# jamesonquinn/Mamba.jl

Hardware: AMD Instinct MI355X
Metric: chain-updates/sec (iters×chains) on rats model at 1/2/4/8 MI355X (higher is better)
Workload: dtype f64

## Files before the change

mamba.jl_amd/csrc/device.h:

```cpp
#pragma once
#if !defined(__HIPCC_RTC__)
#include <hip/hip_runtime.h>
#include <stdint.h>
#endif

#include "mamba_hip.h"
#include "mmb_math.h"
#include "ir_math.h"

#define MMB_MAXB MMB_MAX_BLOCKS

__device__ __forceinline__ bool mmb_inverse_ballot(uint64_t m) {
#if defined(__HIPCC_RTC__)
  return ((m >> (threadIdx.x & 63)) & 1ull) != 0ull;
#else
  return __builtin_amdgcn_inverse_ballot_w64(m);
#endif
}

template <bool B>
struct mmb_bc {
  static constexpr bool value = B;
  constexpr operator bool() const { return B; }
};

__device__ __forceinline__ bool mmb_fast_range(double x) { return x >= 0x1p-700 && x <= 0x1p700; }
__device__ __forceinline__ double mmb_sqrt_inrange(double x) {
  const double y = __builtin_amdgcn_rsq(x);
  double g = x * y, h = 0.5 * y;
  const double r = fma(-h, g, 0.5);
  g = fma(g, r, g);
  h = fma(h, r, h);
  double d = fma(-g, g, x);
  g = fma(d, h, g);
  d = fma(-g, g, x);
  return fma(d, h, g);
}
__device__ __forceinline__ double mmb_rcp_inrange(double y) {
  double r = __builtin_amdgcn_rcp(y);
  double e = fma(-y, r, 1.0);
  r = fma(r, e, r);
  e = fma(-y, r, 1.0);
  r = fma(r, e, r);
  e = fma(-y, r, 1.0);
  return fma(e, r, r);
}
__device__ __forceinline__ void mmb_sqrt_rcp_inrange(double x, double* s, double* rcp) {
  *s = mmb_sqrt_inrange(x);
  *rcp = mmb_rcp_inrange(*s);
}

#define MMB_AMM_STAT_STRIDE 8

struct DBlock {
  int32_t kind, nn, d, transform, form, adapt, batchsize, sigl_diag;
  int32_t nodes[4];
  int32_t emap[4];
  double target, beta, scale;
  double width0;
  const double* width;
  const double* sigl;
  double* t_sigma;
  double* t_accept;
  int32_t* t_m;
  int32_t* t_flags;
  double* t_Mv;
  double* t_Mvv;
  double* t_Ls;
  uint8_t* t_piv;
  double* t_xnext;
  int64_t* t_xtag;
  uint64_t* t_astat;
  double* t_nuts;
  double* t_nfr;
  double* t_hmc;
  int32_t ir_blk;
  int32_t fdgrad;
  const int32_t* sep;
  double sep_eps;
  int32_t gibbs_fam;
  double gibbs_a;
};

struct SweepArgs {
  int32_t K;
  uint32_t chain_offset;
  uint64_t seed;
  int64_t iter0;
  int32_t n_iters;
  int32_t nb;
  int64_t burnin, thin, model_burnin;
  int64_t kept_base;
  int64_t kept_origin;
  double* vals;
  int64_t xepoch;
  unsigned long long* nuts_stat;
  double* draws;
  const double* data0;
  double ig_c;
  double xbar;
  double xm[5];
  double lx[5], ly[5];
  const DBlock* blocks;
  const mmb_ir_node* ir_nodes;
  const int32_t* ir_code;
  const double* ir_const;
  const double* ir_pool;
  const mmb_ir_block* ir_blocks;
  const int32_t* ir_mon;
  int32_t ir_nmon, ir_pmon;
  int32_t ir_vs;
  int32_t ir_red0;
  int32_t ir_amm;
  int32_t ir_lds;
  const int32_t* cperm;
  int32_t wg_offset;
  int32_t wg_stride;
  int32_t amwg_exact;
  int32_t slice_exact;
  int32_t amwg_probe;
};

#define MMB_ORDER_BLOCKS 3
struct OrderArgs {
  const int32_t* flags[MMB_ORDER_BLOCKS];
  int32_t nblk;
  int32_t K;
  int32_t cpw;
  int32_t mode;
  int32_t* perm;
};

__device__ __forceinline__ const DBlock& mmb_block(const DBlock* p, int b) {
#if defined(__HIP_DEVICE_COMPILE__)
  return *(const DBlock*)&((const __attribute__((address_space(4))) DBlock*)p)[b];
#else
  return p[b];
#endif
}

MMB_HD int mmb_tri(int i) { return (i * (i + 1)) >> 1; }
MMB_HD int mmb_slot(int i, int k) { return i >= k ? mmb_tri(i) + k : mmb_tri(k) + i; }

__device__ __forceinline__ void grp_sync() {
  __builtin_amdgcn_fence(__ATOMIC_RELEASE, "wavefront");
  __builtin_amdgcn_wave_barrier();
  __builtin_amdgcn_fence(__ATOMIC_ACQUIRE, "wavefront");
}

template <int CTRL>
__device__ __forceinline__ int dpp_i(int x) {
  return __builtin_amdgcn_mov_dpp(x, CTRL, 0xF, 0xF, true);
}
template <int CTRL>
__device__ __forceinline__ double dpp_d(double x) {
  uint64_t u = mmb_d2u(x);
  int lo = dpp_i<CTRL>((int)(uint32_t)u), hi = dpp_i<CTRL>((int)(uint32_t)(u >> 32));
  return mmb_u2d((uint64_t)(uint32_t)lo | ((uint64_t)(uint32_t)hi << 32));
}
__device__ __forceinline__ int swap16_i(int x) {
  auto r = __builtin_amdgcn_permlane16_swap((unsigned)x, (unsigned)x, false, false);
  return (int)((threadIdx.x & 16) ? r[0] : r[1]);
}
__device__ __forceinline__ double swap16_d(double x) {
// ... 182 lines not shown
```

mamba.jl_amd/csrc/engine.cpp:

```cpp
#include <hip/hip_runtime.h>

#include <algorithm>
#include <cmath>
#include <cstdarg>
#include <cstdio>
#include <cstdlib>
#include <cstring>
#include <map>
#include <string>
#include <type_traits>
#include <vector>

#include "device.h"
#include "models.h"
#include "nuts.h"
#include "logistic.h"
#include "ir.h"
#include "ir_jit.h"

#include <rccl/rccl.h>

hipError_t mmb_launch_sweep(int model, unsigned kinds, const SweepArgs& A, hipStream_t st);
hipError_t mmb_launch_order_chains(const OrderArgs& a, hipStream_t st);
hipError_t mmb_launch_pchol_probe(int n, int d, const double* S, double* L, int32_t* pos, int32_t* info,
// ... 942 lines not shown
int64_t mmb_num_kept(const mmb_engine* e) { return e ? e->n_kept : MMB_E_ARG; }

int64_t mmb_tune_len(const mmb_engine* e) {
  if (!e) return MMB_E_ARG;
  int64_t n = 0;
  for (auto& h : e->blocks) n += h.tune_len;
  return n;
}

static void to_device_layout(const mmb_engine* e, const double* v, double* dv) {
  if (e->model == MMB_MODEL_RATS) {
    std::fill(dv, dv + e->VS, 0.0);
    for (int i = 0; i < 30; ++i) { dv[i] = v[1 + i]; dv[32 + i] = v[33 + i]; }
    dv[64] = v[0]; dv[65] = v[31]; dv[66] = v[32]; dv[67] = v[63]; dv[68] = v[64];
  } else if (e->model == MMB_MODEL_LOGISTIC || e->model == MMB_MODEL_IR) {
    std::fill(dv, dv + e->VS, 0.0);
    for (int i = 0; i < e->P; ++i) dv[i] = v[i];
  } else {
    dv[0] = v[0]; dv[1] = v[1]; dv[2] = v[2]; dv[3] = 0.0;
  }
}
static void from_device_layout(const mmb_engine* e, const double* dv, double* v) {
  if (e->model == MMB_MODEL_RATS) {
    for (int i = 0; i < 30; ++i) { v[1 + i] = dv[i]; v[33 + i] = dv[32 + i]; }
    v[0] = dv[64]; v[31] = dv[65]; v[32] = dv[66]; v[63] = dv[67]; v[64] = dv[68];
  } else if (e->model == MMB_MODEL_LOGISTIC || e->model == MMB_MODEL_IR) {
    for (int i = 0; i < e->P; ++i) v[i] = dv[i];
  } else {
    v[0] = dv[0]; v[1] = dv[1]; v[2] = dv[2];
  }
}

int mmb_set_values(mmb_engine* e, const double* values) {
  if (!e || !values) return fail(e, MMB_E_ARG, "null argument");
  if (!e->d_vals) return fail(e, MMB_E_STATE, "mmb_init_chains not called");
  ++e->xepoch;
  std::vector<double> h((size_t)e->K * e->VS);
  for (int64_t k = 0; k < e->K; ++k) to_device_layout(e, values + k * e->P, h.data() + k * e->VS);
  HIPCHK(e, hipSetDevice(e->device));
  HIPCHK(e, hipMemcpy(e->d_vals, h.data(), h.size() * sizeof(double), hipMemcpyHostToDevice));
  return 0;
}

int mmb_get_values(mmb_engine* e, double* values) {
  if (!e || !values) return fail(e, MMB_E_ARG, "null argument");
  if (!e->d_vals) return fail(e, MMB_E_STATE, "mmb_init_chains not called");
  std::vector<double> h((size_t)e->K * e->VS);
  HIPCHK(e, hipSetDevice(e->device));
  HIPCHK(e, hipStreamSynchronize(e->stream));
  HIPCHK(e, hipMemcpy(h.data(), e->d_vals, h.size() * sizeof(double), hipMemcpyDeviceToHost));
  for (int64_t k = 0; k < e->K; ++k) from_device_layout(e, h.data() + k * e->VS, values + k * e->P);
  return 0;
}

static int upload_blocks(mmb_engine* e) {
  std::vector<DBlock> db(e->blocks.size());
  for (size_t b = 0; b < e->blocks.size(); ++b) {
    BlockHost& h = e->blocks[b];
    DBlock& d = db[b];
    std::memset(&d, 0, sizeof d);
    d.kind = h.spec.sampler;
    d.nn = h.spec.nnodes;
    d.d = h.d;
    d.transform = h.spec.sampler == MMB_SAMPLER_SLICE ? h.spec.transform : 1;
    d.form = h.spec.form;
    d.adapt = h.spec.adapt;
    d.batchsize = h.spec.batchsize;
    d.sigl_diag = h.sigl_diag;
    d.fdgrad = h.spec.gradient != MMB_GRAD_ANALYTIC ? 1 : 0;
    for (int a = 0; a < 4; ++a) d.nodes[a] = a < h.spec.nnodes ? h.spec.nodes[a] : -1;
    int o = 0;
    for (int a = 0; a < h.spec.nnodes && o < 4; ++a) {
      int n = h.spec.nodes[a];
      if (e->model == MMB_MODEL_LINE) {
        if (n == MMB_LINE_BETA) { d.emap[o++] = 0; if (o < 4) d.emap[o++] = 1; }
        else d.emap[o++] = 2;
      } else {
        d.emap[o++] = n;
      }
    }
    d.target = h.spec.target;
    d.beta = h.spec.beta;
    d.scale = h.spec.scale;
    d.width0 = h.tuning.empty() ? 0.0 : h.tuning[0];
    d.width = (h.spec.sampler == MMB_SAMPLER_SLICE && h.tuning.size() > 1) ? h.width : nullptr;
    d.sigl = h.sigl_d;
    d.t_sigma = h.sigma; d.t_accept = h.accept; d.t_m = h.m; d.t_flags = h.flags;
    d.t_Mv = h.Mv; d.t_Mvv = h.Mvv; d.t_Ls = h.Ls; d.t_piv = h.piv; d.t_xnext = h.xnext; d.t_xtag = h.xtag; d.t_nuts = h.nuts; d.t_nfr = h.nfr;
    d.t_astat = h.astat;
    d.t_hmc = h.hmc;
    d.ir_blk = (int32_t)b;
    d.gibbs_a = __builtin_nan("");
    if (e->model == MMB_MODEL_IR && h.spec.sampler == MMB_SAMPLER_GIBBS) {
      const mmb_ir_block& IB = e->ir_blocks[b];
      const int pc = IB.gibbs_expr[0];
      if (IB.gibbs_family != MMB_IR_NORMAL && pc >= 0 && pc + 1 < (int)e->ir_code.size() &&
          (int)((uint32_t)e->ir_code[pc] >> 24) == MMB_IR_OP_CONST && e->ir_code[pc + 1] == MMB_IR_OP_END) {
        const double a = e->ir_const[e->ir_code[pc] & 0xffffff];
        if (a >= 1.0) d.gibbs_a = a;
      }
      d.gibbs_fam = IB.gibbs_family;
    }
    d.sep = h.sep_d;
    d.sep_eps = h.sep_eps;
  }
  if (!e->d_blocks) HIPCHK(e, hipMalloc(&e->d_blocks, MMB_MAX_BLOCKS * sizeof(DBlock)));
  HIPCHK(e, hipMemcpy(e->d_blocks, db.data(), db.size() * sizeof(DBlock), hipMemcpyHostToDevice));
  return 0;
}

template <class T>
static hipError_t dalloc(T** p, size_t n) {
  return hipMalloc((void**)p, std::max<size_t>(n, 1) * sizeof(T));
}

int mmb_init_chains(mmb_engine* e, const double* init, int64_t K, int64_t chain_offset, uint64_t seed) {
  if (!e || !init) return fail(e, MMB_E_ARG, "null argument");
  if (K < 1 || K > (int64_t)1 << 30) return fail(e, MMB_E_ARG, "K out of range");
  if (chain_offset < 0 || chain_offset + K > ((int64_t)1 << 32))
    return fail(e, MMB_E_ARG, "global chain ids must fit in 32 bits");
  if (!e->have_data) return fail(e, MMB_E_STATE, "inputs must be set before inits");
  HIPCHK(e, hipSetDevice(e->device));
  HIPCHK(e, hipStreamSynchronize(e->stream));
  free_dev(e);
  e->K = K;
  e->chain_offset = chain_offset;
  e->seed = seed;
  e->iter = 0;
  e->n_kept = 0;
  HIPCHK(e, dalloc(&e->d_vals, (size_t)K * e->VS));
  e->slice_overflows = 0;
  HIPCHK(e, dalloc(&e->d_nstat, 8));
  HIPCHK(e, hipMemset(e->d_nstat, 0, 8 * sizeof(unsigned long long)));
  const size_t DP = e->DP, TP = e->TP;
  for (auto& h : e->blocks) {
    HIPCHK(e, dalloc(&h.m, K));
    HIPCHK(e, dalloc(&h.flags, K));
    HIPCHK(e, hipMemset(h.m, 0, K * sizeof(int32_t)));
    HIPCHK(e, hipMemset(h.flags, 0, K * sizeof(int32_t)));
    if (h.spec.sampler == MMB_SAMPLER_AMWG) {
      HIPCHK(e, dalloc(&h.sigma, K * DP));
      HIPCHK(e, dalloc(&h.accept, K * DP));
      std::vector<double> sg(K * DP, 0.0);
      for (int64_t k = 0; k < K; ++k)
        for (int i = 0; i < h.d; ++i) sg[k * DP + i] = h.tuning.size() == 1 ? h.tuning[0] : h.tuning[i];
      HIPCHK(e, hipMemcpy(h.sigma, sg.data(), sg.size() * sizeof(double), hipMemcpyHostToDevice));
      HIPCHK(e, hipMemset(h.accept, 0, K * DP * sizeof(double)));
    } else if (h.spec.sampler == MMB_SAMPLER_AMM) {
      HIPCHK(e, dalloc(&h.Mv, K * DP));
      HIPCHK(e, dalloc(&h.Mvv, K * TP));
      HIPCHK(e, dalloc(&h.Ls, K * TP));
      HIPCHK(e, dalloc(&h.piv, K * DP));
      HIPCHK(e, hipMemset(h.Mv, 0, K * DP * sizeof(double)));
      HIPCHK(e, hipMemset(h.Mvv, 0, K * TP * sizeof(double)));
      HIPCHK(e, hipMemset(h.Ls, 0, K * TP * sizeof(double)));
      std::vector<uint8_t> pv(K * DP);
      for (int64_t k = 0; k < K; ++k)
        for (size_t i = 0; i < DP; ++i) pv[k * DP + i] = (uint8_t)i;
      HIPCHK(e, hipMemcpy(h.piv, pv.data(), pv.size(), hipMemcpyHostToDevice));
      HIPCHK(e, dalloc(&h.xnext, K * DP));
      HIPCHK(e, dalloc(&h.xtag, K));
      HIPCHK(e, hipMemset(h.xtag, 0xff, K * sizeof(int64_t)));
      HIPCHK(e, dalloc(&h.astat, K * MMB_AMM_STAT_STRIDE));
      HIPCHK(e, hipMemset(h.astat, 0, K * MMB_AMM_STAT_STRIDE * sizeof(uint64_t)));
      HIPCHK(e, dalloc(&h.sigl_d, (size_t)h.d * h.d));
      HIPCHK(e, hipMemcpy(h.sigl_d, h.sigl.data(), h.sigl.size() * sizeof(double), hipMemcpyHostToDevice));
// ... 1639 lines not shown
```

mamba.jl_amd/csrc/samplers.h:

```cpp
#pragma once
#include "models.h"
#include "hmc.h"
#include "nuts.h"

template <class M>
struct Smp {
  static constexpr int G = M::G, R = M::R, DMAX = M::DMAX, DP = M::DP, TP = M::TP;
  static constexpr int NT = (TP + G - 1) / G;
  using St = typename M::St;
  using Lc = typename M::Lc;

  __device__ __forceinline__ static double predraw(const SweepArgs& A, uint32_t chain, int64_t it,
                                                   const Grp<G>& g) {
    int q = 0;
    for (int t = A.nb; A.nb > 0 && t + A.nb <= 32; t += A.nb) q += g.lane >= t ? 1 : 0;
    const int bl = g.lane - q * A.nb;
    int kind = 0;
    double a = 0.0;
    for (int b = 0; b < A.nb; ++b) {
      const DBlock& B = mmb_block(A.blocks, b);
      double ab = 0.0;
      int k = 0;
      if (B.kind == MMB_SAMPLER_GIBBS) k = M::gibbs_draw_kind(B, &ab);
      else if (B.kind == MMB_SAMPLER_AMM) k = 3;
// ... 221 lines not shown
          grp_sync();
#pragma unroll
          for (int r = 0; r < R; ++r) {
            int e = r * G + g.lane;
            if (!done[r]) {
              double t0 = 0.0, t1 = 0.0;
#pragma unroll
              for (int k = 0; k + 1 < j; k += 2) {
                const double2 pp = *(const double2*)(prow + k);
                t0 = fma(Lrow[r][k], pp.x, t0);
                t1 = fma(Lrow[r][k + 1], pp.y, t1);
              }
              if (j & 1) t0 = fma(Lrow[r][j - 1], prow[j - 1], t0);
              double lij = (mat[mmb_slot(e, p)] - (t0 + t1)) * rinv;
              Lrow[r][j] = lij;
              work[r] = work[r] + lij * lij;
            }
          }
          grp_sync();
        }
      }
    }
    if (rank == d) {
#pragma unroll
      for (int r = 0; r < R; ++r) {
        int e = r * G + g.lane;
        if (e < d) {
          bool before = true;
#pragma unroll
          for (int k = 0; k < DMAX; ++k) {
            if (k < d) {
              const int q = pks[k];
              if (q == e) {
                mat[mmb_tri(e) + e] = Lrow[r][k];
                before = false;
              } else if (before) {
                mat[mmb_slot(e, q)] = Lrow[r][k];
              }
            }
          }
        }
      }
    }
    return rank;
  }

  __device__ __forceinline__ static int pivot_exact(double dl, bool done, const int* pks, int j,
                                                              int d, int* perm, double* val) {
    const int lane = (int)(threadIdx.x & (G - 1));
    if (lane == 0) {
      for (int t = 0; t < d; ++t) perm[t] = t;
      for (int k = 0; k < j; ++k) {
        int q = pks[k], qpos = k;
        for (int t = k; t < d; ++t) if (perm[t] == q) qpos = t;
        int tmp = perm[k]; perm[k] = q; perm[qpos] = tmp;
      }
    }
    grp_sync();
    int mypos = 0x7fffffff;
    for (int t = j; t < d; ++t) if (perm[t] == lane) mypos = t;
    grp_sync();
    double key = done ? -__builtin_inf()
                      : (isnan(dl) ? (mypos == j ? __builtin_inf() : -__builtin_inf()) : dl);
    int pi = (done ? 0x7fff : mypos) << 16 | lane;
    Grp<G> g;
    g.argmax(key, pi);
    const int p = pi & 0xffff;
    *val = g.bcast(dl, p);
    return p;
  }

  __device__ __forceinline__ static int gmax_i32(int x) {
    x = max(x, dpp_i<MMB_DPP_XOR1>(x));
    x = max(x, dpp_i<MMB_DPP_XOR2>(x));
    x = max(x, dpp_i<MMB_DPP_HMIRROR>(x));
    x = max(x, dpp_i<MMB_DPP_MIRROR>(x));
    auto r = __builtin_amdgcn_permlane16_swap((unsigned)x, (unsigned)x, false, false);
    return max((int)r[0], (int)r[1]);
  }

  __device__ __forceinline__ static int pchol32(int d, double* mat, double* prow, int* pks, const Grp<G>& g,
                                                int* pos_out, const DBlock* NB = nullptr,
                                                const SweepArgs& A = SweepArgs{}, int c = 0, uint32_t chain = 0,
                                                int64_t it = 0, int b = 0, int m = 0, int* redo = nullptr) {
    if (d == DMAX)
      return pchol32_impl<true>(d, mat, prow, pks, pos_out, NB, A.seed, A.xepoch, c, chain, it, b, m, redo);
    return pchol32_impl<false>(d, mat, prow, pks, pos_out, NB, A.seed, A.xepoch, c, chain, it, b, m, redo);
  }
  template <bool FULLD>
  __device__ __forceinline__ static int pchol32_impl(int d_arg, double* mat, double* prow, int* pks, int* pos_out,
                                                     const DBlock* NB, uint64_t seed, int64_t xepoch, int c,
                                                     uint32_t chain, int64_t it, int b, int m,
                                                     int* redo_out) {
    const int d = FULLD ? DMAX : d_arg;
    const Grp<G> g;
    constexpr int RI = DMAX;
    const int lane = g.lane;
    const bool hi_half = (threadIdx.x & 32) != 0;
    const bool inb = lane < d;
    const int lc = inb ? lane : 0;
    const double diag0 = inb ? mat[mmb_tri(lane) + lane] : 0.0;
    double work = 0.0;
    double Lrow[DMAX];
#pragma unroll
    for (int k = 0; k < DMAX; ++k) Lrow[k] = 0.0;
    MMB_PROF_START
    bool done = !inb;
    int rank = d;
    int pe = 0;
    bool live = true;
    auto tail = [&]() __attribute__((always_inline)) -> int {
      MMB_PROF_MARK(10, lane)
      if (NB != nullptr && (rank == d || m <= 2 * d)) {
        const mmb_rng rn1 = mmb_rng_make(seed, chain, (uint32_t)(it + 1), (uint32_t)b, MMB_SUB_NORMAL);
        double z1n = 0.0, z2n = 0.0;
        if (inb) mmb_normal_pair(&rn1, (uint32_t)lane, &z1n, &z2n);
        double a = 0.0;
        if (inb) a = fma(NB->sigl[lane * d + lane], z1n, a);
        if (m > 2 * d) {
          double y = 0.0;
          const double zs = swap16_d(z2n);
          const bool row0 = (lane & 16) == 0;
          const double zA = row0 ? z2n : zs, zB = row0 ? zs : z2n;
#pragma unroll
          for (int k = 0; k < DMAX; ++k) fmac_rowbc_n(y, k < 16 ? zA : zB, Lrow[k], k & 15);
          a = NB->beta * a + (1.0 - NB->beta) * y;
        }
        if (inb) NB->t_xnext[(size_t)c * DP + lane] = a;
        if (lane == 0) NB->t_xtag[c] = (xepoch << 32) | (int64_t)(uint32_t)(it + 1);
      }
      MMB_PROF_MARK(11, lane)
      if (rank == d && inb) {
        const int base = mmb_tri(pe);
#pragma unroll
        for (int k = 0; k < DMAX; ++k) {
          double* dst = k <= pe ? mat + base + k : prow + lane;
          *dst = Lrow[k];
        }
      }
      MMB_PROF_MARK(12, lane)
      *pos_out = pe;
      return rank;
    };
    if (!inb) work = __builtin_inf();
    const uint32_t mat_lds = (uint32_t)(uintptr_t)(__attribute__((address_space(3))) double*)mat;
    int hmask = hi_half ? -1 : 0;
    asm volatile("" : "+v"(hmask));
    constexpr int KEY_LO = 0x14300000;
    constexpr double BIG = 0x1p700;
    auto pass = [&](auto checked_c) __attribute__((always_inline)) -> bool {
      constexpr bool CHECKED = decltype(checked_c)::value;
      double apiv = 1.0;
      double inf_s = __builtin_inf();
      asm volatile("" : "+s"(inf_s));
#pragma unroll
      for (int j = 0; j < DMAX; ++j) {
        if (live && j < d) {
          const double dl = diag0 - work;
          const int key = (int)(mmb_d2u(dl) >> 32);
          const int mx = gmax_i32(key);
          const uint64_t eq = __ballot(key == mx);
          uint32_t elo = (uint32_t)eq, ehi = (uint32_t)(eq >> 32);
          int p = 0;
          const uint64_t negm = __ballot(mx < 0);
          bool pos = mmb_inverse_ballot(~negm);
          bool fast = true;
          if constexpr (!CHECKED) {
            const int plo = __builtin_ctz(elo | 0x80000000u), phi = __builtin_ctz(ehi | 0x80000000u);
            p = plo ^ ((plo ^ phi) & hmask);
          } else {
            const uint64_t act = __builtin_amdgcn_read_exec();
            const uint64_t bad = __ballot(!(dl < BIG));
            const uint64_t big = __ballot(key >= KEY_LO);
            const uint64_t neg = __ballot(mx < 0);
            uint32_t alo = (uint32_t)act, ahi = (uint32_t)(act >> 32);
            uint32_t nlo = (uint32_t)neg, nhi = (uint32_t)(neg >> 32), blo = (uint32_t)big, bhi = (uint32_t)(big >> 32);
            asm("" : "+s"(elo), "+s"(ehi), "+s"(alo), "+s"(ahi));
            asm("" : "+s"(nlo), "+s"(nhi), "+s"(blo), "+s"(bhi));
            const bool ok_lo = alo == 0 || nlo != 0 || ((elo & (elo - 1)) == 0 && blo != 0);
            const bool ok_hi = ahi == 0 || nhi != 0 || ((ehi & (ehi - 1)) == 0 && bhi != 0);
            fast = bad == 0 && ok_lo && ok_hi;
            if (fast) {
              const int plo = __builtin_ctz(elo | 0x80000000u), phi = __builtin_ctz(ehi | 0x80000000u);
              p = plo ^ ((plo ^ phi) & hmask);
            } else {
              double val;
              p = pivot_exact(dl, done, pks, j, d, (int*)prow, &val);
              pos = val > 0.0;
            }
          }
          if (CHECKED && !pos) {
            live = false;
          } else {
            const bool piv = CHECKED ? lane == p : mmb_inverse_ballot(eq & ~negm);
            if (piv) {
              if constexpr (CHECKED) pks[j] = p;
              else apiv = dl;
              if (j + 1 < d) {
#pragma unroll
                for (int k = 0; k + 1 < j; k += 2) *(double2*)(prow + k) = make_double2(Lrow[k], Lrow[k + 1]);
                if (j & 1) prow[j - 1] = Lrow[j - 1];
              }
              double ajj, rinv;
              if (fast) {
                mmb_sqrt_rcp_inrange(dl, &ajj, &rinv);
              } else {
                ajj = sqrt(dl);
                rinv = 1.0 / ajj;
              }
              prow[RI] = rinv;
              Lrow[j] = ajj;
              pe = j;
// ... 23 lines not shown
                }
              }
              const double lij = (sig - (t0 + t1)) * rinv;
              const bool keep = CHECKED ? done : work == inf_s;
              work = work + lij * lij;
              if (!keep) Lrow[j] = lij;
            }
            grp_sync();
            if (!CHECKED) live = live && pos;
          }
        }
      }
      if constexpr (CHECKED) {
        return false;
      } else {
        done = work == inf_s;
        const bool inr = apiv >= 0x1p-700 && apiv <= 0x1p700;
        uint64_t need = __ballot(inb && (done ? !inr : isnan(diag0 - work)));
        const uint64_t dn = __ballot(done && inb);
        const int mpe = gmax_i32((done && inb) ? pe : -1);
        const uint64_t act = __builtin_amdgcn_read_exec();
        const int m0 = __builtin_amdgcn_readlane(mpe, 0), m1 = __builtin_amdgcn_readlane(mpe, 32);
        if ((uint32_t)act != 0u && __builtin_popcount((uint32_t)dn) != m0 + 1) need |= 1ull;
        if ((act >> 32) != 0u && __builtin_popcount((uint32_t)(dn >> 32)) != m1 + 1) need |= 1ull << 32;
        return need != 0;
      }
    };
    if (__builtin_expect(pass(mmb_bc<false>{}), 0)) {
      if (redo_out) *redo_out = 1;
      work = inb ? 0.0 : __builtin_inf();
#pragma unroll
      for (int k = 0; k < DMAX; ++k) Lrow[k] = 0.0;
      done = !inb;
      pe = 0;
      live = true;
      (void)pass(mmb_bc<true>{});
    }
    const uint64_t dn = __ballot(done && inb);
    rank = __builtin_popcount(hi_half ? (uint32_t)(dn >> 32) : (uint32_t)dn);
    return tail();
  }

  static constexpr bool IKTAB = (G == 32);
  __device__ __forceinline__ static uint16_t* ik_table() {
    __shared__ uint16_t tab[IKTAB ? TP : 1];
    return tab;
  }
  __device__ __forceinline__ static void ik_fill() {
    if constexpr (IKTAB) {
      for (int t = (int)threadIdx.x; t < TP; t += (int)blockDim.x) {
        int i, k;
        slot_ik(t, i, k);
        ik_table()[t] = (uint16_t)(i << 8 | k);
      }
    }
  }
  __device__ __forceinline__ static void slot_ik(int s, int& i, int& k) {
    int ii = (int)((sqrtf((float)(8 * s + 1)) - 1.0f) * 0.5f);
    ii += (mmb_tri(ii + 1) <= s) ? 1 : 0;
    ii -= (mmb_tri(ii) > s) ? 1 : 0;
    i = ii;
    k = s - mmb_tri(ii);
  }

  __device__ __forceinline__ static void amm_count(const DBlock& B, int c, int d, int rank, int redo,
                                                   const Grp<G>& g) {
    const int st = rank < d ? rank + 1 : d;
    int ws = st;
    if constexpr (G == 32) {
      const uint64_t act = __builtin_amdgcn_read_exec();
      const int s0 = __builtin_amdgcn_readlane(st, 0), s1 = __builtin_amdgcn_readlane(st, 32);
      ws = max((uint32_t)act != 0u ? s0 : 0, (act >> 32) != 0u ? s1 : 0);
    }
    if (g.lane == 0) {
      uint64_t* a = B.t_astat + (size_t)c * MMB_AMM_STAT_STRIDE;
      (void)__hip_atomic_fetch_add(a + 0, (uint64_t)1, __ATOMIC_RELAXED, __HIP_MEMORY_SCOPE_AGENT);
      if (rank == d) (void)__hip_atomic_fetch_add(a + 1, (uint64_t)1, __ATOMIC_RELAXED, __HIP_MEMORY_SCOPE_AGENT);
      (void)__hip_atomic_fetch_add(a + 2, (uint64_t)rank, __ATOMIC_RELAXED, __HIP_MEMORY_SCOPE_AGENT);
      (void)__hip_atomic_fetch_add(a + 3, (uint64_t)ws, __ATOMIC_RELAXED, __HIP_MEMORY_SCOPE_AGENT);
      if (redo) (void)__hip_atomic_fetch_add(a + 4, (uint64_t)redo, __ATOMIC_RELAXED, __HIP_MEMORY_SCOPE_AGENT);
    }
  }

  static constexpr bool CARRY = (G == 32 && R == 1);
  static constexpr bool POSFORM = (G == 32 && R == 1);
  __device__ __forceinline__ static int64_t xtag(const SweepArgs& A, int64_t it) {
    return (A.xepoch << 32) | (int64_t)(uint32_t)it;
  }
  __device__ __forceinline__ static void amm(const SweepArgs& A, const DBlock& B, int c, uint32_t chain,
                             int64_t it, int b, const mmb_rng& rn,
                             const mmb_rng& ru, bool adapt, St& s, const Lc& l, const Grp<G>& g,
                             double* lds, double upre, typename M::PrepCache& pk) {
    const int d = B.d;
    const int T = mmb_tri(d);
    double* mat = lds;
    double* z2s = lds + TP;
    double* vvs = z2s + DP;
    double* mvs = vvs + DP;
    int* ia = (int*)(mvs + DP);
    double v[R], x[R], z1[R], z2[R], mv[R];
    MMB_PROF_START
    M::unlist(B, s, g.lane, v);
    int m = B.t_m[c];
    int fl = B.t_flags[c];
#pragma unroll
    for (int r = 0; r < R; ++r) {
      int e = r * G + g.lane;
      mv[r] = e < d ? B.t_Mv[(size_t)c * DP + e] : 0.0;
    }
    const bool fresh = adapt && !(fl & 1);
    bool carried = false;
    if constexpr (CARRY) carried = B.t_xtag != nullptr && !fresh && B.t_xtag[c] == xtag(A, it);
    if (fresh) {
      m = 0;
      fl = (fl | 2) & ~4;
#pragma unroll
      for (int r = 0; r < R; ++r) mv[r] = v[r];
    }
    fl = adapt ? (fl | 1) : (fl & ~1);
    MMB_PROF_MARK(1, g.lane)
    if (carried) {
#pragma unroll
      for (int r = 0; r < R; ++r) {
        const int e = r * G + g.lane;
        x[r] = e < d ? B.t_xnext[(size_t)c * DP + e] : 0.0;
      }
    } else {
#pragma unroll
    for (int r = 0; r < R; ++r) {
      int e = r * G + g.lane;
      if (e < d) mmb_normal_pair(&rn, (uint32_t)e, &z1[r], &z2[r]);
      else { z1[r] = 0.0; z2[r] = 0.0; }
    }
    if (!B.sigl_diag) {
#pragma unroll
      for (int r = 0; r < R; ++r) {
        int e = r * G + g.lane;
        if (e < d) vvs[e] = z1[r];
      }
      grp_sync();
    }
#pragma unroll
    for (int r = 0; r < R; ++r) {
      int e = r * G + g.lane;
      double a = 0.0;
      if (e < d) {
        if (B.sigl_diag) {
          a = fma(B.sigl[e * d + e], z1[r], a);
        } else {
          for (int k = 0; k <= e; ++k) a = fma(B.sigl[e * d + k], vvs[k], a);
        }
      }
      x[r] = a;
    }
    if (m > 2 * d) {
      double y[R];
#pragma unroll
      for (int r = 0; r < R; ++r) y[r] = 0.0;
      if (fl & 4) {
        grp_sync();
        const double* Ls = B.t_Ls + (size_t)c * TP;
        double lt[NT];
#pragma unroll
        for (int u = 0; u < NT; ++u) lt[u] = (u * G + g.lane < T) ? Ls[u * G + g.lane] : 0.0;
#pragma unroll
        for (int u = 0; u < NT; ++u)
          if (u * G + g.lane < T) mat[u * G + g.lane] = lt[u];
        if constexpr (POSFORM) {
          const int e = g.lane;
          const int pe = e < d ? (int)B.t_piv[(size_t)c * DP + e] : 0;
          if (e < d) z2s[e] = z2[0];
          grp_sync();
          const double* row = mat + mmb_tri(pe);
          double a = 0.0;
#pragma unroll
          for (int k = 0; k < DMAX; ++k)
            if (k < d) a = k <= pe ? fma(row[k], z2s[k], a) : a;
          if (e < d) y[0] = a;
        } else {
        uint32_t pw[DP / 4];
        const uint32_t* pvw = (const uint32_t*)(B.t_piv + (size_t)c * DP);
#pragma unroll
        for (int w = 0; w < DP / 4; ++w) pw[w] = pvw[w];
#pragma unroll
        for (int r = 0; r < R; ++r) {
          int e = r * G + g.lane;
          if (e < d) z2s[e] = z2[r];
        }
        grp_sync();
#pragma unroll
        for (int r = 0; r < R; ++r) {
          const int e = r * G + g.lane;
          int pe = 0;
#pragma unroll
          for (int k = 0; k < DMAX; ++k)
            if (k < d && (int)((pw[k >> 2] >> (8 * (k & 3))) & 0xffu) == e) pe = k;
          double a = 0.0;
#pragma unroll
          for (int k = 0; k < DMAX; ++k) {
            if (k < d) {
              const int q = (int)((pw[k >> 2] >> (8 * (k & 3))) & 0xffu);
              const double m_ = mat[mmb_slot(e, q)];
              const double z_ = z2s[k];
              a = (k < pe) ? fma(m_, z_, a) : a;
            }
          }
          if (e < d) y[r] = fma(mat[mmb_tri(e) + e], z2s[pe], a);
        }
        }
      }
#pragma unroll
      for (int r = 0; r < R; ++r) x[r] = B.beta * x[r] + (1.0 - B.beta) * y[r];
    }
    }
#pragma unroll
    for (int r = 0; r < R; ++r) x[r] = x[r] + v[r];
    MMB_PROF_MARK(2, g.lane)
    const typename M::Prep pc = M::prep(B, s, g, pk);
    MMB_PROF_MARK(0, g.lane)
    double lx, lv;
    M::logf_p2(A, B, pc, s, l, g, x, v, lx, lv);
    const double ua = G == 32 ? upre : mmb_uniform(&ru, 0u);
    if (ua < mmb_exp(lx - lv)) {
#pragma unroll
      for (int r = 0; r < R; ++r) v[r] = x[r];
    }
    MMB_PROF_MARK(3, g.lane)
    if (adapt) {
      m += 1;
      const double p = (double)m / ((double)m + 1.0);
      const double q = 1.0 - p;
      if (fl & 2) {
#pragma unroll
        for (int r = 0; r < R; ++r) mv[r] = p * v[r] + q * v[r];
        fl &= ~2;
      } else {
#pragma unroll
        for (int r = 0; r < R; ++r) mv[r] = p * mv[r] + q * v[r];
      }
      grp_sync();
      double2* vm = (double2*)vvs;
#pragma unroll
      for (int r = 0; r < R; ++r) {
        int e = r * G + g.lane;
        if (e < d) vm[e] = make_double2(v[r], mv[r]);
      }
      const double cc = (B.scale * B.scale / (double)d) / p;
      double* Mvv = B.t_Mvv + (size_t)c * TP;
      double vold[R];
      if (fresh) {
        M::unlist(B, s, g.lane, vold);
#pragma unroll
        for (int r = 0; r < R; ++r) {
          int e = r * G + g.lane;
          if (e < d) z2s[e] = vold[r];
        }
      }
      grp_sync();
      double lt[NT];
#pragma unroll
      for (int u = 0; u < NT; ++u) lt[u] = (!fresh && u * G + g.lane < TP) ? Mvv[u * G + g.lane] : 0.0;
      double* const Mvv_l = Mvv + g.lane;
      double* const mat_l = mat + g.lane;
      auto slots = [&](auto fresh_c) {
        constexpr bool FRESH = decltype(fresh_c)::value;
        int li0 = g.lane;
        asm volatile("" : "+v"(li0));
#pragma unroll
        for (int u = 0; u < NT; ++u) {
          const int t = u * G + g.lane;
          if ((u + 1) * G <= TP || t < TP) {
            int i, k;
            if constexpr (IKTAB) {
              const int li = li0;
              const int w = ik_table()[li + u * G];
              i = w >> 8;
              k = w & 255;
            } else {
              int ti = t;
              asm volatile("" : "+v"(ti));
              slot_ik(ti, i, k);
            }
            const double2 a = vm[k], bi = vm[i];
            const double old = FRESH ? z2s[i] * z2s[k] : lt[u];
            const double nv = p * old + (q * a.x) * bi.x;
            lt[u] = nv;
            mat_l[u * G] = cc * (nv - a.y * bi.y);
          }
        }
      };
      if (fresh) slots(mmb_bc<true>{});
      else slots(mmb_bc<false>{});
#pragma unroll
      for (int u = 0; u < NT; ++u)
        if ((u + 1) * G <= TP || u * G + g.lane < TP) Mvv_l[u * G] = lt[u];
      grp_sync();
#pragma unroll
      for (int r = 0; r < R; ++r) {
        int e = r * G + g.lane;
        if (e < d) B.t_Mv[(size_t)c * DP + e] = mv[r];
      }
      if (g.lane == 0) { B.t_m[c] = m; B.t_flags[c] = fl; }
      M::relist(B, s, g, v);
      M::stash(lds, s, g.lane);
      int* pks = (int*)z2s;
      grp_sync();
      MMB_PROF_MARK(4, g.lane)
      int rank;
      int redo = 0;
      const bool carry = CARRY && B.t_xtag != nullptr && B.sigl_diag;
      int pe = 0;
      if constexpr (G == 32 && R == 1)
        rank = pchol32(d, mat, (double*)ia, pks, g, &pe, carry ? &B : nullptr, A, c, chain, it, b, m, &redo);
      else
        rank = pchol(d, mat, (double*)ia, pks, g);
      grp_sync();
      MMB_PROF_MARK(5, g.lane)
      if (B.t_astat != nullptr) amm_count(B, c, d, rank, redo, g);
      if (rank == d) {
        double* Ls = B.t_Ls + (size_t)c * TP;
#pragma unroll
        for (int u = 0; u < NT; ++u)
          if (u * G + g.lane < T) Ls[u * G + g.lane] = mat[u * G + g.lane];
        uint8_t* pv = B.t_piv + (size_t)c * DP;
        if constexpr (POSFORM) {
          if (g.lane < d) pv[g.lane] = (uint8_t)pe;
        } else {
          for (int k = g.lane; k < d; k += G) pv[k] = (uint8_t)pks[k];
        }
        if (g.lane == 0) B.t_flags[c] = fl | 4;
      }
      M::unstash(lds, s, g.lane);
      grp_sync();
      MMB_PROF_MARK(6, g.lane)
      return;
    }
#pragma unroll
    for (int r = 0; r < R; ++r) {
      int e = r * G + g.lane;
      if (e < d) B.t_Mv[(size_t)c * DP + e] = mv[r];
    }
    if (g.lane == 0) { B.t_m[c] = m; B.t_flags[c] = fl; }
    grp_sync();
    M::relist(B, s, g, v);
  }

  __device__ __forceinline__ static void slice_overflow(const SweepArgs& A, const Grp<G>& g) {
    if (g.lane == 0) atomicAdd(&A.nuts_stat[3], 1ull);
  }
  __device__ __forceinline__ static double width(const DBlock& B, int e) {
    return B.width ? B.width[e] : B.width0;
  }
  struct UWin {
    double u;
    uint32_t base;
  };
  __device__ __forceinline__ static double uwin_next(const mmb_rng& ru, UWin& w, uint32_t k, const Grp<G>& g) {
    if (k - w.base >= (uint32_t)G) {
      w.base = k;
      w.u = mmb_uniform(&ru, k + (uint32_t)g.lane);
    }
    const int src = (int)(threadIdx.x & 63 & ~(G - 1)) + (int)(k - w.base);
    return __shfl(w.u, src, 64);
  }
  __device__ __forceinline__ static void slice_uni_cand(const SweepArgs& A, const DBlock& B, const mmb_rng& ru,
                                                        St& s, const Lc& l, const Grp<G>& g, double* lds) {
    constexpr int SD = M::SLICE_CAND_D;
    constexpr int NC = M::SLICE_NC, LPC = 32 / NC;
    constexpr uint32_t LEAD = NC == 2 ? 0x00010001u : NC == 4 ? 0x01010101u : 0x11111111u;
    static_assert(MMB_SLICE_MAX_SHRINK % NC == 0, "rounds of candidates end at the cap");
    const int d = B.d;
    double x[R];
    M::unlist(B, s, g.lane, x);
    typename M::SCtx cx;
    M::slice_cand_prep(A, B, s, l, g, lds, cx);
    double logf0 = M::slice_logf0(A, B, s, l, g, x, cx);
    double lo = 0.0, up = 0.0;
    if (g.lane < d) {
      const double w = width(B, g.lane);
      lo = x[0] - w * mmb_uniform(&ru, (uint32_t)g.lane);
      up = lo + w;
    }
    typename M::SMemo memo;
    double xu[SD], lou[SD], upu[SD];
#pragma unroll
    for (int a = 0; a < SD; ++a) {
      xu[a] = a < d ? g.bcast(x[0], a) : 0.0;
      lou[a] = a < d ? g.bcast(lo, a) : 0.0;
      upu[a] = a < d ? g.bcast(up, a) : 0.0;
    }
    uint32_t k = (uint32_t)d;
    UWin uw{0.0, 0xffffffffu - (uint32_t)G};
    const int q = g.lane / LPC;
    const int gbase = (int)(threadIdx.x & 63) & ~(G - 1);
    for (int e = 0; e < d; ++e) {
      const double p0 = logf0 + mmb_log(uwin_next(ru, uw, k++, g));
      double xo = xu[0], lo_ = lou[0], up_ = upu[0];
#pragma unroll
      for (int a = 1; a < SD; ++a)
        if (a == e) { xo = xu[a]; lo_ = lou[a]; up_ = upu[a]; }
      double xn = 0.0, lfn = 0.0;
      for (uint32_t j0 = 0;; j0 += NC) {
        double cand[NC];
#pragma unroll
        for (int t = 0; t < NC; ++t) {
          const double cv = lo_ + (up_ - lo_) * uwin_next(ru, uw, k + j0 + (uint32_t)t, g);
          cand[t] = cv;
          if (cv < xo) lo_ = cv;
          else up_ = cv;
        }
        double mine = cand[0];
#pragma unroll
        for (int t = 1; t < NC; ++t) mine = q == t ? cand[t] : mine;
        double xv[SD];
#pragma unroll
        for (int a = 0; a < SD; ++a) xv[a] = a == e ? mine : xu[a];
        const double lp = M::slice_cand_logf(A, B, s, cx, xv, g.lane, memo);
        const bool hit = !(lp < p0) && j0 + (uint32_t)q + 1u <= (uint32_t)MMB_SLICE_MAX_SHRINK;
        const uint64_t bal = __ballot(hit && (g.lane & (LPC - 1)) == 0);
        const uint32_t hb = (uint32_t)(bal >> gbase) & LEAD;
        if (hb != 0u) {
          const int qs = __builtin_ctz(hb) / LPC;
          xn = cand[0];
#pragma unroll
          for (int t = 1; t < NC; ++t) xn = qs == t ? cand[t] : xn;
// ... 262 lines not shown
```

mamba.jl_amd/csrc/sweep.h:

```cpp
#pragma once
#include "samplers.h"
#include "ir.h"

#ifdef MMB_PHASE_PROF
extern __device__ unsigned long long mmb_prof[32];
#endif
#ifdef MMB_WAVE_TIMES
#define MMB_WT_MAX 65536
extern __device__ unsigned long long mmb_wt[3 * MMB_WT_MAX];
#endif

#ifndef MMB_SWEEP_WAVES
#define MMB_SWEEP_WAVES 4
#endif
#ifndef MMB_IR_WAVES
#define MMB_IR_WAVES 2
#endif
template <int MODEL>
constexpr int sweep_waves() {
  return MODEL == MMB_MODEL_RATS ? MMB_SWEEP_WAVES : MODEL == MMB_MODEL_IR ? MMB_IR_WAVES : 1;
}

template <int MODEL, unsigned KINDS>
__device__ __forceinline__ void sweep_body(const SweepArgs& A) {
  using M = Mdl<MODEL>;
  using S = Smp<M>;
  constexpr int G = M::G;
  extern __shared__ __attribute__((aligned(16))) double smem[];
  if constexpr ((KINDS >> MMB_SAMPLER_AMM) & 1u) {
    S::ik_fill();
    __syncthreads();
  }
#ifdef MMB_IR_POOL_LDS
  if constexpr (MODEL == MMB_MODEL_IR) {
    double* ps = mmb_ir_pool_s();
    for (int t = (int)threadIdx.x; t < MMB_IR_POOL_LDS; t += (int)blockDim.x) ps[t] = A.ir_pool[t];
    __syncthreads();
  }
#endif
  const unsigned wg = blockIdx.x * (unsigned)A.wg_stride + (unsigned)A.wg_offset;
  const int slot = (int)((wg * blockDim.x + threadIdx.x) / G);
#ifdef MMB_WAVE_TIMES
  const uint64_t _wt0 = __builtin_amdgcn_s_memrealtime();
  const int _wid = (int)((wg * blockDim.x + threadIdx.x) >> 6);
#endif
  if (slot >= A.K) return;
  const int c = A.cperm != nullptr ? A.cperm[slot] : slot;
  Grp<G> g;
  double* lds = smem + (size_t)(threadIdx.x / G) * M::lds_stride(A);
  typename M::St s;
  typename M::Lc l;
  M::load(A, c, g.lane, s, l, lds);
  const uint32_t chain = A.chain_offset + (uint32_t)c;
#ifdef MMB_PHASE_PROF
  if ((threadIdx.x & 63) == 0)
    for (int i = 0; i < 16; ++i) mmb_prof_lds()[i] = 0;
#endif
  constexpr bool PREDRAW = G == 32 && (KINDS & ((1u << MMB_SAMPLER_GIBBS) | (1u << MMB_SAMPLER_AMM))) != 0u;
  int pre0 = 0;
  double pre = 0.0;
  typename M::PrepCache pk = M::prep_cache(lds);
  for (int step = 0; step < A.n_iters; ++step) {
    const int64_t it = A.iter0 + 1 + step;
#ifdef MMB_PHASE_PROF
    const uint64_t _it0 = __builtin_amdgcn_s_memtime();
#endif
    if constexpr (PREDRAW) {
      if (__builtin_expect(pre0 == 0, 0)) {
        MMB_PROF_START
        pre = S::predraw(A, chain, it, g);
        MMB_PROF_MARK(15, g.lane)
      }
    }
    for (int b = 0; b < A.nb; ++b) {
      const DBlock& B = mmb_block(A.blocks, b);
      const mmb_rng rn = mmb_rng_make(A.seed, chain, (uint32_t)it, (uint32_t)b, MMB_SUB_NORMAL);
      const mmb_rng ru = mmb_rng_make(A.seed, chain, (uint32_t)it, (uint32_t)b, MMB_SUB_UNIFORM);
      const bool adapt = B.adapt == MMB_ADAPT_ALL ? true
                         : B.adapt == MMB_ADAPT_BURNIN ? (it <= A.model_burnin) : false;
      switch (B.kind) {
        case MMB_SAMPLER_AMWG:
          if constexpr ((KINDS >> MMB_SAMPLER_AMWG) & 1u) {
            MMB_PROF_START
            S::amwg(A, B, c, rn, ru, adapt, s, l, g, pk);
            MMB_PROF_MARK(13, g.lane)
          }
          break;
        case MMB_SAMPLER_AMM:
          if constexpr ((KINDS >> MMB_SAMPLER_AMM) & 1u) S::amm(A, B, c, chain, it, b, rn, ru, adapt, s, l, g, lds,
                                                                        G == 32 ? S::lane_value(pre, pre0 + b) : 0.0, pk);
          break;
        case MMB_SAMPLER_SLICE:
          if constexpr ((KINDS >> MMB_SAMPLER_SLICE) & 1u) {
            MMB_PROF_START
            if (B.form == MMB_SLICE_UNIVARIATE) S::slice_uni(A, B, ru, s, l, g, lds);
            else S::slice_multi(A, B, ru, s, l, g, lds);
            MMB_PROF_MARK(14, g.lane)
          }
          break;
        case MMB_SAMPLER_NUTS:
          if constexpr ((KINDS >> MMB_SAMPLER_NUTS) & 1u) S::nuts(A, B, c, it, b, s, g);
          break;
        case MMB_SAMPLER_HMC:
          if constexpr ((KINDS >> MMB_SAMPLER_HMC) & 1u) S::template hmc<false>(A, B, c, rn, ru, s, g);
          break;
        case MMB_SAMPLER_MALA:
          if constexpr ((KINDS >> MMB_SAMPLER_MALA) & 1u) S::template hmc<true>(A, B, c, rn, ru, s, g);
          break;
        case MMB_SAMPLER_GIBBS: if constexpr ((KINDS >> MMB_SAMPLER_GIBBS) & 1u) {
          const mmb_rng gn = mmb_rng_make(A.seed, chain, (uint32_t)it, (uint32_t)b, MMB_SUB_GAMMA_N);
          const mmb_rng gu = mmb_rng_make(A.seed, chain, (uint32_t)it, (uint32_t)b, MMB_SUB_GAMMA_U);
          MMB_PROF_START
          M::gibbs(A, B, s, l, g, &rn, &gn, &gu, G == 32 ? S::lane_value(pre, pre0 + b) : 0.0);
          MMB_PROF_MARK(7, g.lane)
        }
          break;
        default:
          break;
      }
      M::prep_wrote(pk, B);
    }
#ifdef MMB_PHASE_PROF
    if ((threadIdx.x & 63) == 0) {
      mmb_prof_lds()[8] += __builtin_amdgcn_s_memtime() - _it0;
      mmb_prof_lds()[9] += 1;
    }
#endif
    pre0 += A.nb;
    if (pre0 + A.nb > 32) pre0 = 0;
    if (A.draws && it > A.burnin && (it - A.burnin) % A.thin == 0) {
      const int64_t row = (it - A.burnin) / A.thin - 1 - A.kept_origin;
      M::write_draws(A, s, g, row, c);
    }
  }
  M::store(A, c, g.lane, s);
#ifdef MMB_WAVE_TIMES
  if ((threadIdx.x & 63) == 0 && _wid < MMB_WT_MAX) {
    const uint64_t _wt1 = __builtin_amdgcn_s_memrealtime();
    if (mmb_wt[3 * _wid] == 0) mmb_wt[3 * _wid] = _wt0;
    mmb_wt[3 * _wid + 1] = _wt1;
    mmb_wt[3 * _wid + 2] += _wt1 - _wt0;
  }
#endif
#ifdef MMB_PHASE_PROF
  if ((threadIdx.x & 63) == 0)
    for (int i = 0; i < 16; ++i) atomicAdd(&mmb_prof[i], mmb_prof_lds()[i]);
#endif
}

#ifndef MMB_RATS_BLOCK
#define MMB_RATS_BLOCK 256
#endif
template <int MODEL, unsigned KINDS>
__global__ __launch_bounds__(MODEL == MMB_MODEL_RATS && MMB_RATS_BLOCK > 256 ? MMB_RATS_BLOCK : 256,
                             sweep_waves<MODEL>()) void sweep_kernel(const SweepArgs A) {
  sweep_body<MODEL, KINDS>(A);
}

constexpr unsigned K_ALL = (1u << MMB_SAMPLER_AMWG) | (1u << MMB_SAMPLER_AMM) |
                         (1u << MMB_SAMPLER_SLICE) | (1u << MMB_SAMPLER_GIBBS);
constexpr unsigned K_GRAD = (1u << MMB_SAMPLER_NUTS) | (1u << MMB_SAMPLER_HMC) | (1u << MMB_SAMPLER_MALA);
constexpr unsigned K_ALL_GRAD = K_ALL | K_GRAD;
constexpr unsigned K_GIBBS_AMM = (1u << MMB_SAMPLER_AMM) | (1u << MMB_SAMPLER_GIBBS);
constexpr unsigned K_SLICE_AMWG = (1u << MMB_SAMPLER_AMWG) | (1u << MMB_SAMPLER_SLICE);
constexpr unsigned K_IR = (1u << MMB_SAMPLER_AMWG) | (1u << MMB_SAMPLER_AMM) | (1u << MMB_SAMPLER_SLICE) |
                         (1u << MMB_SAMPLER_GIBBS) | K_GRAD;
```

Baseline: 152.7 million.

## Keep AMM per-chain scalar state in lane registers across sweep iterations

Per-chain AMM scalars (iteration count, flags, carry tag, acceptance statistics) now live in a lane-distributed register word for the whole sweep. They are read with readlane and written back once when the kernel ends, instead of being loaded and stored in global memory on every iteration, and the per-iteration atomic stat increments are batched into one atomic add at the end. It also precomputes scale^2/d on the host and zeroes an LDS slot at kernel start. The cost is more register pressure and extra bookkeeping logic, and the fast path only applies when the group size is 32 with R==1 and there are at most four AMM blocks.

After: 153.6 million, median of 6. No clear change (+0.6%).

```diff
diff --git a/mamba.jl_amd/csrc/device.h b/mamba.jl_amd/csrc/device.h
--- a/mamba.jl_amd/csrc/device.h
+++ b/mamba.jl_amd/csrc/device.h
@@ -80,6 +80,7 @@
   double sep_eps;
   int32_t gibbs_fam;
   double gibbs_a;
+  double scale2d;
 };
 
 struct SweepArgs {
diff --git a/mamba.jl_amd/csrc/engine.cpp b/mamba.jl_amd/csrc/engine.cpp
--- a/mamba.jl_amd/csrc/engine.cpp
+++ b/mamba.jl_amd/csrc/engine.cpp
@@ -1048,6 +1048,11 @@
     d.target = h.spec.target;
     d.beta = h.spec.beta;
     d.scale = h.spec.scale;
+    {
+      volatile double s2 = h.spec.scale * h.spec.scale;
+      volatile double s2d = s2 / (double)(h.d > 0 ? h.d : 1);
+      d.scale2d = s2d;
+    }
     d.width0 = h.tuning.empty() ? 0.0 : h.tuning[0];
     d.width = (h.spec.sampler == MMB_SAMPLER_SLICE && h.tuning.size() > 1) ? h.width : nullptr;
     d.sigl = h.sigl_d;
diff --git a/mamba.jl_amd/csrc/samplers.h b/mamba.jl_amd/csrc/samplers.h
--- a/mamba.jl_amd/csrc/samplers.h
+++ b/mamba.jl_amd/csrc/samplers.h
@@ -327,16 +327,17 @@
   __device__ __forceinline__ static int pchol32(int d, double* mat, double* prow, int* pks, const Grp<G>& g,
                                                 int* pos_out, const DBlock* NB = nullptr,
                                                 const SweepArgs& A = SweepArgs{}, int c = 0, uint32_t chain = 0,
-                                                int64_t it = 0, int b = 0, int m = 0, int* redo = nullptr) {
+                                                int64_t it = 0, int b = 0, int m = 0, int* redo = nullptr,
+                                                bool wtag = true, bool* wrote = nullptr) {
     if (d == DMAX)
-      return pchol32_impl<true>(d, mat, prow, pks, pos_out, NB, A.seed, A.xepoch, c, chain, it, b, m, redo);
-    return pchol32_impl<false>(d, mat, prow, pks, pos_out, NB, A.seed, A.xepoch, c, chain, it, b, m, redo);
+      return pchol32_impl<true>(d, mat, prow, pks, pos_out, NB, A.seed, A.xepoch, c, chain, it, b, m, redo, wtag, wrote);
+    return pchol32_impl<false>(d, mat, prow, pks, pos_out, NB, A.seed, A.xepoch, c, chain, it, b, m, redo, wtag, wrote);
   }
   template <bool FULLD>
   __device__ __forceinline__ static int pchol32_impl(int d_arg, double* mat, double* prow, int* pks, int* pos_out,
                                                      const DBlock* NB, uint64_t seed, int64_t xepoch, int c,
                                                      uint32_t chain, int64_t it, int b, int m,
-                                                     int* redo_out) {
+                                                     int* redo_out, bool wtag, bool* wrote) {
     const int d = FULLD ? DMAX : d_arg;
     const Grp<G> g;
     constexpr int RI = DMAX;
@@ -372,7 +373,8 @@
           a = NB->beta * a + (1.0 - NB->beta) * y;
         }
         if (inb) NB->t_xnext[(size_t)c * DP + lane] = a;
-        if (lane == 0) NB->t_xtag[c] = (xepoch << 32) | (int64_t)(uint32_t)(it + 1);
+        if (wtag && lane == 0) NB->t_xtag[c] = (xepoch << 32) | (int64_t)(uint32_t)(it + 1);
+        if (wrote) *wrote = true;
       }
       MMB_PROF_MARK(11, lane)
       if (rank == d && inb) {
@@ -562,6 +564,71 @@
     }
   }
 
+  static constexpr bool SSREG = (G == 32 && R == 1);
+  static constexpr int SS_MAX = 4;
+  __device__ __forceinline__ static uint32_t ss_get(uint32_t ss, int i) {
+    const uint32_t a = (uint32_t)__builtin_amdgcn_readlane((int)ss, i);
+    const uint32_t b = (uint32_t)__builtin_amdgcn_readlane((int)ss, i + 32);
+    return (threadIdx.x & 32) ? b : a;
+  }
+  __device__ __forceinline__ static bool ss_load(const SweepArgs& A, int c, const Grp<G>& g, uint32_t& ss) {
+    int na = 0;
+    for (int b = 0; b < A.nb; ++b) na += mmb_block(A.blocks, b).kind == MMB_SAMPLER_AMM ? 1 : 0;
+    if (na > SS_MAX) return false;
+    const int32_t* pw = nullptr;
+    const int64_t* pt = nullptr;
+    int o = 0;
+    for (int b = 0; b < A.nb; ++b) {
+      const DBlock& B = mmb_block(A.blocks, b);
+      if (B.kind != MMB_SAMPLER_AMM) continue;
+      const int k = g.lane - 8 * o;
+      pw = k == 0 ? B.t_m + c : k == 1 ? B.t_flags + c : pw;
+      pt = (k == 2 && B.t_xtag != nullptr) ? B.t_xtag + c : pt;
+      ++o;
+    }
+    const int32_t w = pw != nullptr ? *pw : 0;
+    const int64_t t = pt != nullptr ? *pt : -1;
+    ss = pt != nullptr ? (t == xtag(A, A.iter0 + 1) ? 1u : 0u) : (uint32_t)w;
+    return true;
+  }
+  __device__ __forceinline__ static void ss_store(const SweepArgs& A, int c, const Grp<G>& g, uint32_t ss,
+                                                  int64_t last) {
+    int o = 0;
+    for (int b = 0; b < A.nb; ++b) {
+      const DBlock& B = mmb_block(A.blocks, b);
+      if (B.kind != MMB_SAMPLER_AMM) continue;
+      const int k = g.lane - 8 * o;
+      if (k == 0) B.t_m[c] = (int32_t)ss;
+      else if (k == 1) B.t_flags[c] = (int32_t)ss;
+      else if (k == 2) {
+        if (B.t_xtag != nullptr) B.t_xtag[c] = xtag(A, ss != 0u ? last + 1 : last);
+      } else if (k >= 3 && k < 8) {
+        if (B.t_astat != nullptr && ss != 0u)
+          (void)__hip_atomic_fetch_add(B.t_astat + (size_t)c * MMB_AMM_STAT_STRIDE + (k - 3), (uint64_t)ss,
+                                       __ATOMIC_RELAXED, __HIP_MEMORY_SCOPE_AGENT);
+      }
+      ++o;
+    }
+  }
+  __device__ __forceinline__ static void ss_count(uint32_t& ss, int slot0, int d, int rank, int redo,
+                                                  const Grp<G>& g) {
+    const int st = rank < d ? rank + 1 : d;
+    const uint64_t act = __builtin_amdgcn_read_exec();
+    const int s0 = __builtin_amdgcn_readlane(st, 0), s1 = __builtin_amdgcn_readlane(st, 32);
+    const int ws = max((uint32_t)act != 0u ? s0 : 0, (act >> 32) != 0u ? s1 : 0);
+    const int k = g.lane - slot0;
+    int inc = k == 3 ? 1 : 0;
+    inc = k == 4 ? (rank == d ? 1 : 0) : inc;
+    inc = k == 5 ? rank : inc;
+    inc = k == 6 ? ws : inc;
+    inc = k == 7 ? redo : inc;
+    ss += (uint32_t)inc;
+  }
+
+  __device__ __forceinline__ static void amm_lds_init(double* lds, int lane) {
+    if constexpr (G == 32 && R == 1) (lds + TP + 3 * DP)[lane] = 0.0;
+  }
+
   static constexpr bool CARRY = (G == 32 && R == 1);
   static constexpr bool POSFORM = (G == 32 && R == 1);
   __device__ __forceinline__ static int64_t xtag(const SweepArgs& A, int64_t it) {
@@ -570,7 +637,8 @@
   __device__ __forceinline__ static void amm(const SweepArgs& A, const DBlock& B, int c, uint32_t chain,
                              int64_t it, int b, const mmb_rng& rn,
                              const mmb_rng& ru, bool adapt, St& s, const Lc& l, const Grp<G>& g,
-                             double* lds, double upre, typename M::PrepCache& pk) {
+                             double* lds, double upre, typename M::PrepCache& pk, uint32_t& ss, int slot0) {
+    const bool on = SSREG && slot0 >= 0;
     const int d = B.d;
     const int T = mmb_tri(d);
     double* mat = lds;
@@ -581,8 +649,16 @@
     double v[R], x[R], z1[R], z2[R], mv[R];
     MMB_PROF_START
     M::unlist(B, s, g.lane, v);
-    int m = B.t_m[c];
-    int fl = B.t_flags[c];
+    int m, fl;
+    bool cbit = false;
+    if (on) {
+      m = (int)ss_get(ss, slot0);
+      fl = (int)ss_get(ss, slot0 + 1);
+      cbit = ss_get(ss, slot0 + 2) != 0u;
+    } else {
+      m = B.t_m[c];
+      fl = B.t_flags[c];
+    }
 #pragma unroll
     for (int r = 0; r < R; ++r) {
       int e = r * G + g.lane;
@@ -590,22 +666,24 @@
     }
     const bool fresh = adapt && !(fl & 1);
     bool carried = false;
-    if constexpr (CARRY) carried = B.t_xtag != nullptr && !fresh && B.t_xtag[c] == xtag(A, it);
+    if constexpr (CARRY) {
+      if (on) carried = cbit && !fresh;
+      else carried = B.t_xtag != nullptr && !fresh && B.t_xtag[c] == xtag(A, it);
+    }
+    if (carried) {
+#pragma unroll
+      for (int r = 0; r < R; ++r) {
+        const int e = r * G + g.lane;
+        x[r] = e < d ? B.t_xnext[(size_t)c * DP + e] : 0.0;
+      }
+    }
     if (fresh) {
       m = 0;
       fl = (fl | 2) & ~4;
-#pragma unroll
-      for (int r = 0; r < R; ++r) mv[r] = v[r];
     }
     fl = adapt ? (fl | 1) : (fl & ~1);
     MMB_PROF_MARK(1, g.lane)
-    if (carried) {
-#pragma unroll
-      for (int r = 0; r < R; ++r) {
-        const int e = r * G + g.lane;
-        x[r] = e < d ? B.t_xnext[(size_t)c * DP + e] : 0.0;
-      }
-    } else {
+    if (!carried) {
 #pragma unroll
     for (int r = 0; r < R; ++r) {
       int e = r * G + g.lane;
@@ -725,7 +803,7 @@
         int e = r * G + g.lane;
         if (e < d) vm[e] = make_double2(v[r], mv[r]);
       }
-      const double cc = (B.scale * B.scale / (double)d) / p;
+      const double cc = B.scale2d / p;
       double* Mvv = B.t_Mvv + (size_t)c * TP;
       double vold[R];
       if (fresh) {
@@ -780,7 +858,13 @@
         int e = r * G + g.lane;
         if (e < d) B.t_Mv[(size_t)c * DP + e] = mv[r];
       }
-      if (g.lane == 0) { B.t_m[c] = m; B.t_flags[c] = fl; }
+      if (on) {
+        ss = g.lane == slot0 ? (uint32_t)m : ss;
+        ss = g.lane == slot0 + 1 ? (uint32_t)fl : ss;
+      } else if (g.lane == 0) {
+        B.t_m[c] = m;
+        B.t_flags[c] = fl;
+      }
       M::relist(B, s, g, v);
       M::stash(lds, s, g.lane);
       int* pks = (int*)z2s;
@@ -790,13 +874,22 @@
       int redo = 0;
       const bool carry = CARRY && B.t_xtag != nullptr && B.sigl_diag;
       int pe = 0;
+      bool wrote = false;
       if constexpr (G == 32 && R == 1)
-        rank = pchol32(d, mat, (double*)ia, pks, g, &pe, carry ? &B : nullptr, A, c, chain, it, b, m, &redo);
+        rank = pchol32(d, mat, (double*)ia, pks, g, &pe, carry ? &B : nullptr, A, c, chain, it, b, m, &redo, !on,
+                       &wrote);
       else
         rank = pchol(d, mat, (double*)ia, pks, g);
       grp_sync();
       MMB_PROF_MARK(5, g.lane)
-      if (B.t_astat != nullptr) amm_count(B, c, d, rank, redo, g);
+      if (on) {
+        const uint32_t f4 = rank == d ? 4u : 0u;
+        ss = g.lane == slot0 + 1 ? ss | f4 : ss;
+        ss = g.lane == slot0 + 2 ? (wrote ? 1u : 0u) : ss;
+        if (B.t_astat != nullptr) ss_count(ss, slot0, d, rank, redo, g);
+      } else if (B.t_astat != nullptr) {
+        amm_count(B, c, d, rank, redo, g);
+      }
       if (rank == d) {
         double* Ls = B.t_Ls + (size_t)c * TP;
 #pragma unroll
@@ -808,7 +901,7 @@
         } else {
           for (int k = g.lane; k < d; k += G) pv[k] = (uint8_t)pks[k];
         }
-        if (g.lane == 0) B.t_flags[c] = fl | 4;
+        if (!on && g.lane == 0) B.t_flags[c] = fl | 4;
       }
       M::unstash(lds, s, g.lane);
       grp_sync();
@@ -820,7 +913,14 @@
       int e = r * G + g.lane;
       if (e < d) B.t_Mv[(size_t)c * DP + e] = mv[r];
     }
-    if (g.lane == 0) { B.t_m[c] = m; B.t_flags[c] = fl; }
+    if (on) {
+      ss = g.lane == slot0 ? (uint32_t)m : ss;
+      ss = g.lane == slot0 + 1 ? (uint32_t)fl : ss;
+      ss = g.lane == slot0 + 2 ? 0u : ss;
+    } else if (g.lane == 0) {
+      B.t_m[c] = m;
+      B.t_flags[c] = fl;
+    }
     grp_sync();
     M::relist(B, s, g, v);
   }
diff --git a/mamba.jl_amd/csrc/sweep.h b/mamba.jl_amd/csrc/sweep.h
--- a/mamba.jl_amd/csrc/sweep.h
+++ b/mamba.jl_amd/csrc/sweep.h
@@ -29,6 +29,8 @@
   extern __shared__ __attribute__((aligned(16))) double smem[];
   if constexpr ((KINDS >> MMB_SAMPLER_AMM) & 1u) {
     S::ik_fill();
+    if (MODEL != MMB_MODEL_IR || A.ir_amm > 0)
+      S::amm_lds_init(smem + (size_t)(threadIdx.x / G) * M::lds_stride(A), (int)(threadIdx.x & (G - 1)));
     __syncthreads();
   }
 #ifdef MMB_IR_POOL_LDS
@@ -60,8 +62,13 @@
   int pre0 = 0;
   double pre = 0.0;
   typename M::PrepCache pk = M::prep_cache(lds);
+  constexpr bool SSREG = S::SSREG && ((KINDS >> MMB_SAMPLER_AMM) & 1u) != 0u;
+  uint32_t ss = 0;
+  bool ss_on = false;
+  if constexpr (SSREG) ss_on = S::ss_load(A, c, g, ss);
   for (int step = 0; step < A.n_iters; ++step) {
     const int64_t it = A.iter0 + 1 + step;
+    int amm_slot = ss_on ? 0 : -1;
 #ifdef MMB_PHASE_PROF
     const uint64_t _it0 = __builtin_amdgcn_s_memtime();
 #endif
@@ -87,8 +94,11 @@
           }
           break;
         case MMB_SAMPLER_AMM:
-          if constexpr ((KINDS >> MMB_SAMPLER_AMM) & 1u) S::amm(A, B, c, chain, it, b, rn, ru, adapt, s, l, g, lds,
-                                                                        G == 32 ? S::lane_value(pre, pre0 + b) : 0.0, pk);
+          if constexpr ((KINDS >> MMB_SAMPLER_AMM) & 1u) {
+            S::amm(A, B, c, chain, it, b, rn, ru, adapt, s, l, g, lds, G == 32 ? S::lane_value(pre, pre0 + b) : 0.0,
+                   pk, ss, amm_slot);
+            if (amm_slot >= 0) amm_slot += 8;
+          }
           break;
         case MMB_SAMPLER_SLICE:
           if constexpr ((KINDS >> MMB_SAMPLER_SLICE) & 1u) {
@@ -134,6 +144,9 @@
     }
   }
   M::store(A, c, g.lane, s);
+  if constexpr (SSREG) {
+    if (ss_on) S::ss_store(A, c, g, ss, A.iter0 + A.n_iters);
+  }
 #ifdef MMB_WAVE_TIMES
   if ((threadIdx.x & 63) == 0 && _wid < MMB_WT_MAX) {
     const uint64_t _wt1 = __builtin_amdgcn_s_memrealtime();
```
